# evanmayer/effex

Measured on AMD Instinct MI355X. Metric: 2-ant FX correlator throughput (PFB+FFT+X, integrated), higher is better.
Workload: dtype f32; 1 GPU; configs[1]: 2-antenna FX, num_samp=262144, ntaps=4, nchan=4096, 10000 integration frames per GPU per step; frames_per_gpu=10000, frames_total=10000, resident_frames=10000, num_samp=262144, nchan=4096, ntaps=4, n_ant=2, sample_definition=one complex sample per antenna stream, reduce_transport=none (single rank), library=effex_amd/csrc/libfxcorr.so

## Files before the change

### effex_amd/csrc/fx_fused4096.h

```cpp
#pragma once
#include "fx_math.h"

#if defined(__HIP_DEVICE_COMPILE__)
#define FXC_SCHED_FENCE() __builtin_amdgcn_sched_barrier(0)
#else
#define FXC_SCHED_FENCE() ((void)0)
#endif

namespace fxc {
namespace fused {

FX_HD cf lds_load(const cf* p) {
#if defined(__HIP_DEVICE_COMPILE__)
    typedef const volatile __attribute__((address_space(3))) unsigned long long* lds_u64_ptr;
    const unsigned long long u = *(lds_u64_ptr)(p);
    cf r;
    r.x = __uint_as_float((unsigned)(u & 0xffffffffull));
    r.y = __uint_as_float((unsigned)(u >> 32));
    return r;
#else
    return *p;
#endif
}

FX_HD f4 lds_load4(const f4* p) {
#if defined(__HIP_DEVICE_COMPILE__)
    typedef float lds_v4f __attribute__((ext_vector_type(4)));
    typedef const volatile __attribute__((address_space(3))) lds_v4f* lds_v4f_ptr;
    const lds_v4f u = *(lds_v4f_ptr)(p);
    f4 r;
    r.x = u[0]; r.y = u[1]; r.z = u[2]; r.w = u[3];
    return r;
#else
    return *p;
#endif
}

constexpr int kN = 4096;
constexpr int kT = 4;
constexpr int kThreads = 512;
constexpr int kPlaneRow = 288;
constexpr int kPlane = 16 * kPlaneRow;
constexpr int kAntPlanes = 2 * kPlane;
constexpr int kRegionBytes = 2 * kAntPlanes * 4;
constexpr int kAccPerThread = 8;
#ifndef FXC_FIR_GROUP
#define FXC_FIR_GROUP 4
#endif
constexpr int kFirGroup = FXC_FIR_GROUP;

constexpr int kLdsRegion = 0;
constexpr int kLdsWin = kLdsRegion + kRegionBytes;
constexpr int kLdsTw2 = kLdsWin + kN * 16;
constexpr int kLdsBytes = kLdsTw2 + 256 * 8;

FX_HD int branch_of_thread(int t) {
    const int l = t & 63, wv = (t >> 6) & 3;
    return ((l >> 1) & 15) + 16 * ((l & 1) | ((l >> 5) << 1) | (wv << 2));
}
FX_HD int thread_of_branch(int j) { return ((j >> 4) & 1) | ((j & 15) << 1) | (j & 0xE0); }

struct LaneStore {
#if defined(__HIP_DEVICE_COMPILE__)
    unsigned m0;
#else
    float* at;
#endif
};

FX_HD LaneStore lane_store_begin(cf* region, int base_dw, int lane) {
    LaneStore ls;
#if defined(__HIP_DEVICE_COMPILE__)
    typedef __attribute__((address_space(3))) cf* lptr_t;
    (void)lane;
    ls.m0 = __builtin_amdgcn_readfirstlane((unsigned)(size_t)(lptr_t)region + 4u * (unsigned)base_dw);
    asm volatile("s_nop 0" : : "{m0}"(ls.m0));
#else
    ls.at = reinterpret_cast<float*>(region) + base_dw + lane;
#endif
    return ls;
}

template <int DW>
FX_HD void lane_store(const LaneStore& ls, float val) {
    static_assert(DW >= 0 && 4 * DW < 65536, "16-bit immediate");
#if defined(__HIP_DEVICE_COMPILE__)
    asm volatile("ds_write_addtid_b32 %0 offset:%1" : : "v"(val), "n"(4 * DW), "{m0}"(ls.m0));
#else
    ls.at[DW] = val;
#endif
}

FX_HD void lane_store_end() {
#if defined(__HIP_DEVICE_COMPILE__)
    asm volatile("s_waitcnt lgkmcnt(0)" : : : "memory");
#endif
}

template <int K>
struct KConst { static constexpr int value = K; };
template <class Sink>
FX_HD void dft16_b_stream_ct(cf (&v)[16], Sink&& sink) {
    dft4(v[0], v[1], v[2], v[3]);
    sink(KConst<0>{}, v[0]); sink(KConst<4>{}, v[1]); sink(KConst<8>{}, v[2]); sink(KConst<12>{}, v[3]);
    dft4_scaled_c_bd(v[4], v[5], v[6], v[7]);
    sink(KConst<1>{}, v[4]); sink(KConst<5>{}, v[5]); sink(KConst<9>{}, v[6]); sink(KConst<13>{}, v[7]);
    dft4_bd_scaled(v[8], v[9], v[10], v[11]);
    sink(KConst<2>{}, v[8]); sink(KConst<6>{}, v[9]); sink(KConst<10>{}, v[10]); sink(KConst<14>{}, v[11]);
    dft4_scaled_c_bd(v[12], v[13], v[14], v[15]);
    sink(KConst<3>{}, v[12]); sink(KConst<7>{}, v[13]); sink(KConst<11>{}, v[14]); sink(KConst<15>{}, v[15]);
}

struct State {
    cf h[4][16];
    cf tw1[16];
    cf acc[kAccPerThread];
    cf tw2[16];
};

template <int PH>
FX_HD void state_reset_history(State& s) {
#pragma unroll
    for (int d = 1; d < 4; ++d)
#pragma unroll
        for (int r = 0; r < 16; ++r) s.h[(PH + d) & 3][r] = mk(0.f, 0.f);
}

FX_HD void state_reset_all(State& s) {
    state_reset_history<0>(s);
#pragma unroll
    for (int q = 0; q < kAccPerThread; ++q) s.acc[q] = mk(0.f, 0.f);
}

struct RangeWalk {
    int c, i;
    int left;
    int row;
    int n_pts;
    int seg, seg_left;
    int seg_jump;
    int unit, in_row;
    int row_step;
    int row_off;
    bool rows_are_chunks;
    bool lead;
};

struct RangeSplit {
    int rounds, n_full, n_tail, rows_rounds, n_rows;
};

FX_HD RangeSplit range_split(int g, int n_chunks, int seg, int unit, bool rows_are_chunks) {
    RangeSplit r;
    r.rounds = n_chunks / (g * seg);
    r.n_full = r.rounds * g * seg;
    r.n_tail = n_chunks - r.n_full;
    r.rows_rounds = rows_are_chunks ? r.n_full : g * ((r.rounds * seg + unit - 1) / unit);
    r.n_rows = r.rows_rounds + r.n_tail + g;
    return r;
}

FX_HD RangeWalk range_walk_rounds(int b, int g, int n_chunks, int n_pts, int seg,
                                   int unit, bool rows_are_chunks) {
    const RangeSplit sp = range_split(g, n_chunks, seg, unit, rows_are_chunks);
    RangeWalk w;
    w.c = b * seg;
    w.i = 0;
    w.left = sp.rounds * seg * n_pts;
    w.n_pts = n_pts;
    w.seg = w.seg_left = seg;
    w.seg_jump = (g - 1) * seg;
    w.unit = rows_are_chunks ? 1 : unit;
    w.in_row = 0;
    w.rows_are_chunks = rows_are_chunks;
    w.row_off = 0;
    w.row_step = g;
    w.row = rows_are_chunks ? w.c : b;
    w.lead = false;
    return w;
}

FX_HD RangeWalk range_walk_tail(int b, int g, int n_chunks, int n_pts, int seg,
                                 int unit, bool rows_are_chunks) {
    const RangeSplit sp = range_split(g, n_chunks, seg, unit, rows_are_chunks);
    RangeWalk w;
    const int n_frames = sp.n_tail * n_pts;
    const int f0 = range_begin(b, n_frames, g);
    w.left = range_begin(b + 1, n_frames, g) - f0;
    w.c = sp.n_full + f0 / n_pts;
    w.i = f0 % n_pts;
    w.n_pts = n_pts;
    w.seg = 1;
    w.seg_left = 1;
    w.seg_jump = 0;
    w.unit = 1;
    w.in_row = 0;
    w.rows_are_chunks = true;
    w.row_off = sp.rows_rounds - sp.n_full;
    w.row_step = 0;
    w.lead = w.i != 0;
    w.row = w.lead ? sp.rows_rounds + sp.n_tail + b : w.c + w.row_off;
    return w;
}

FX_HD bool range_walk_row_ends(const RangeWalk& w) {
    return w.left == 1 || (w.i + 1 == w.n_pts && w.in_row + 1 == w.unit);
}

FX_HD void range_walk_prefetch(const RangeWalk& w, int& pc, int& pi) {
    pc = w.c;
    pi = w.i;
    if (w.left > 1 && ++pi == w.n_pts) {
        pi = 0;
        pc += 1 + (w.seg_left == 1 ? w.seg_jump : 0);
    }
}

FX_HD void range_walk_advance(RangeWalk& w, bool row_ended) {
    if (++w.i == w.n_pts) {
        w.i = 0;
        w.c += 1;
        if (--w.seg_left == 0) {
            w.c += w.seg_jump;
            w.seg_left = w.seg;
        }
        w.in_row += 1;
    }
    w.left -= 1;
    if (row_ended) {
        w.in_row = 0;
        w.row = w.rows_are_chunks ? w.c + w.row_off : w.row + w.row_step;
    }
}

FX_HD int sample_offset(int j, int r) { return (kN - 1) - j - 256 * r; }

template <int PH, int G = kFirGroup, bool PIN = false>
FX_HD void phase1_fir_col(const State& s, const f4* win, int col, cf (&v)[16]) {
    const int j = col;
    const cf (&x0)[16] = s.h[PH];
    const cf (&x1)[16] = s.h[(PH + 3) & 3];
    const cf (&x2)[16] = s.h[(PH + 2) & 3];
    const cf (&x3)[16] = s.h[(PH + 1) & 3];
    constexpr int NG = 16 / G;
    f4 w[2][G];
#pragma unroll
    for (int q = 0; q < G; ++q) w[0][q] = PIN ? lds_load4(win + q * 256 + j) : win[q * 256 + j];
#pragma unroll
    for (int g = 0; g < NG; ++g) {
        if (g < NG - 1) {
#pragma unroll
            for (int q = 0; q < G; ++q) {
                const f4* at = win + (G * (g + 1) + q) * 256 + j;
                w[(g + 1) & 1][q] = PIN ? lds_load4(at) : *at;
            }
        }
        FXC_SCHED_FENCE();
#pragma unroll
        for (int q = 0; q < G; ++q) {
            const int r = G * g + q;
            const f4 t = w[g & 1][q];
            cf a = cscale(x0[r], t.x);
            a = cfma(t.y, x1[r], a);
            a = cfma(t.z, x2[r], a);
            v[r] = cfma(t.w, x3[r], a);
        }
#if defined(__HIP_DEVICE_COMPILE__)
        if (PIN) {
#pragma unroll
            for (int q = 0; q < G; ++q) asm volatile("" : "+v"(v[G * g + q].x), "+v"(v[G * g + q].y));
        }
#endif
        FXC_SCHED_FENCE();
    }
}

template <int PH, int G = kFirGroup>
FX_HD void phase1_fir(const State& s, const f4* win, int tid, cf (&v)[16]) {
    phase1_fir_col<PH, G>(s, win, tid & 255, v);
}

FX_HD cf tw1_of(const cf (&pw2)[4], int k1) {
    cf w = mk(1.f, 0.f);
    bool have = false;
#pragma unroll
    for (int b = 0; b < 4; ++b) {
        if (k1 & (1 << b)) {
            w = have ? cmul(w, pw2[b]) : pw2[b];
            have = true;
        }
    }
    return w;
}

template <bool LEAN_TW = false>
FX_HD void phase1_finish_store(const State& s, cf (&v)[16], cf* region, int tid) {
    const int t = thread_of_branch(tid & 255);
    const LaneStore ls = lane_store_begin(region, (tid >> 8) * kAntPlanes + (t & 0xC0), t & 63);
    cf pw2[4] = {s.tw1[1], s.tw1[2], s.tw1[4], s.tw1[8]};
#if defined(__HIP_DEVICE_COMPILE__)
    if (LEAN_TW) {
#pragma unroll
        for (int b = 0; b < 4; ++b) asm volatile("" : "+v"(pw2[b].x), "+v"(pw2[b].y));
    }
#endif
    dft16_b_stream_ct(v, [&](auto k, cf val) {
        constexpr int k1 = decltype(k)::value;
        if (k1 > 0) val = cmul(val, LEAN_TW ? tw1_of(pw2, k1) : s.tw1[k1]);
        lane_store<k1 * kPlaneRow>(ls, val.x);
        lane_store<kPlane + k1 * kPlaneRow>(ls, val.y);
    });
    lane_store_end();
}

FX_HD void state_load_twiddles(State& s, const cf* tw1_table, int tid) {
    const int j = tid & 255;
#pragma unroll
    for (int k1 = 0; k1 < 16; ++k1) s.tw1[k1] = tw1_table[k1 * 256 + j];
}

FX_HD void phase2_load(cf* region, int tid, cf (&v)[16]) {
    const int l = tid & 63, wave = tid >> 6;
    const int ant = l >> 5, k1 = 2 * wave + ((l >> 4) & 1), j0 = l & 15;
    const float* row = reinterpret_cast<const float*>(region) + ant * kAntPlanes + k1 * kPlaneRow + 2 * j0;
#pragma unroll
    for (int u = 0; u < 8; ++u) {
        const cf re = lds_load(reinterpret_cast<const cf*>(row + 32 * u));
        const cf im = lds_load(reinterpret_cast<const cf*>(row + kPlane + 32 * u));
        v[2 * u] = mk(re.x, im.x);
        v[2 * u + 1] = mk(re.y, im.y);
    }
}

FX_HD void phase2_twiddle(cf (&v)[16], const cf* tw2, int tid) {
    const int j0 = tid & 15;
    cf t[2][4];
#pragma unroll
    for (int q = 1; q < 4; ++q) t[0][q] = lds_load(tw2 + q * 16 + j0);
#pragma unroll
    for (int g = 0; g < 4; ++g) {
        if (g < 3) {
#pragma unroll
            for (int q = 0; q < 4; ++q) t[(g + 1) & 1][q] = lds_load(tw2 + (4 * (g + 1) + q) * 16 + j0);
        }
        FXC_SCHED_FENCE();
#pragma unroll
        for (int q = 0; q < 4; ++q) {
            const int q1 = 4 * g + q;
            if (q1 > 0) v[q1] = cmul(v[q1], t[g & 1][q]);
        }
        FXC_SCHED_FENCE();
    }
}

#ifndef FXC_TW2_RESIDENT
#define FXC_TW2_RESIDENT 10
#endif
constexpr int kTw2Resident = FXC_TW2_RESIDENT;
static_assert(kTw2Resident >= 0 && kTw2Resident <= 15, "q1 = 1 .. 15");
FX_HD void state_load_twiddles2(State& s, const cf* tw2_table, int tid) {
    const int j0 = tid & 15;
#pragma unroll
    for (int q1 = 1; q1 <= kTw2Resident; ++q1) s.tw2[q1] = tw2_table[q1 * 16 + j0];
}

FX_HD void phase2_twiddle_fetch(cf (&t)[16], const cf* tw2, int tid) {
    const int j0 = tid & 15;
#pragma unroll
    for (int q1 = kTw2Resident + 1; q1 < 16; ++q1) t[q1] = lds_load(tw2 + q1 * 16 + j0);
}

FX_HD cf cmul_tw(cf a, cf b) {
    return mk(__builtin_fmaf(a.x, b.x, -(a.y * b.y)), __builtin_fmaf(a.y, b.x, a.x * b.y));
}

FX_HD void phase2_twiddle_reg(cf (&v)[16], const State& s, const cf (&t)[16]) {
#pragma unroll
    for (int q1 = 1; q1 <= kTw2Resident; ++q1) v[q1] = cmul_tw(v[q1], s.tw2[q1]);
#pragma unroll
    for (int q1 = kTw2Resident + 1; q1 < 16; ++q1) v[q1] = cmul_tw(v[q1], t[q1]);
}

constexpr int kStripeHi = kPlane + 32;
constexpr int stripe_of(int q1) { return (q1 >> 3) * kStripeHi + (q1 & 7) * 66; }

template <int Q1>
FX_HD void phase2_store_from(const LaneStore& ls, const cf (&v)[16]) {
    lane_store<stripe_of(Q1)>(ls, v[Q1].x);
    lane_store<stripe_of(Q1) + kAntPlanes>(ls, v[Q1].y);
    if constexpr (Q1 < 15) phase2_store_from<Q1 + 1>(ls, v);
}

FX_HD void phase2_store(const cf (&v)[16], cf* region, int tid) {
    const LaneStore ls = lane_store_begin(region, (tid >> 6) * 2 * kPlaneRow, tid & 63);
    phase2_store_from<0>(ls, v);
    lane_store_end();
}

FX_HD void phase3_load(cf* region, int tid, cf (&v)[16]) {
    const int l = tid & 63, wave = tid >> 6, q1 = l & 15;
    const float* row = reinterpret_cast<const float*>(region) + wave * 2 * kPlaneRow + stripe_of(q1) + (l >> 4) * 16;
#pragma unroll
    for (int u = 0; u < 8; ++u) {
        const cf re = lds_load(reinterpret_cast<const cf*>(row + 2 * u));
        const cf im = lds_load(reinterpret_cast<const cf*>(row + kAntPlanes + 2 * u));
        v[2 * u] = mk(re.x, im.x);
        v[2 * u + 1] = mk(re.y, im.y);
    }
}

FX_HD void xacc(State& s, int q, cf a, cf b) { s.acc[q] = cmulc_acc(s.acc[q], a, b); }

FX_HD int bin_of(int tid, int q) {
    const int l = tid & 63, wave = tid >> 6;
    const int k1 = 2 * wave + ((l >> 4) & 1), q1 = l & 15, q2 = q + 8 * (l >> 5);
    return k1 + 16 * q1 + 256 * q2;
}

FX_HD int slot_of_bin(int k) {
    const int k1 = k & 15, q1 = (k >> 4) & 15, q2 = k >> 8;
    const int l = (q2 >> 3) * 32 + (k1 & 1) * 16 + q1;
    const int tid = (k1 >> 1) * 64 + l;
    return (q2 & 7) * kThreads + tid;
}

FX_HD int lane_specpos(int tid) {
    const int l = tid & 63, wave = tid >> 6;
    return (2 * wave + ((l >> 4) & 1)) * 16 + (l & 15);
}

FX_HD int specpos(int lane_l, int q2) { return (q2 >> 1) * 512 + 2 * lane_l + (q2 & 1); }
FX_HD int specpos_of_bin(int k) { return specpos((k & 15) * 16 + ((k >> 4) & 15), k >> 8); }

}
}
```

### effex_amd/csrc/k_fused4096.h

```cpp
#pragma once

namespace {

__device__ __forceinline__ void wave_sync() {
    __builtin_amdgcn_fence(__ATOMIC_RELEASE, "wavefront");
    __builtin_amdgcn_wave_barrier();
    __builtin_amdgcn_fence(__ATOMIC_ACQUIRE, "wavefront");
}

__device__ __forceinline__ void permlane32_swap(cf& a, cf& b) {
    auto rx = __builtin_amdgcn_permlane32_swap(__float_as_uint(a.x), __float_as_uint(b.x), false, false);
    auto ry = __builtin_amdgcn_permlane32_swap(__float_as_uint(a.y), __float_as_uint(b.y), false, false);
    a = fxc::mk(__uint_as_float(rx[0]), __uint_as_float(ry[0]));
    b = fxc::mk(__uint_as_float(rx[1]), __uint_as_float(ry[1]));
}

typedef unsigned v2u32 __attribute__((ext_vector_type(2)));
typedef unsigned v4u32 __attribute__((ext_vector_type(4)));
#ifndef FXC_LOAD_AUX_U8
#define FXC_LOAD_AUX_U8 2
#endif
#ifndef FXC_LOAD_AUX
#define FXC_LOAD_AUX 2
#endif
#ifndef FXC_PAIR_SOFF
#define FXC_PAIR_SOFF 1
#endif
struct FetchBase {
    const cf* base;
    __amdgpu_buffer_rsrc_t rs, rs_odd;
};
__device__ __forceinline__ void fetch_base_set(FetchBase& fb, const cf* chunk_base, unsigned chunk_bytes) {
    fb.base = chunk_base;
    fb.rs = __builtin_amdgcn_make_buffer_rsrc(const_cast<cf*>(chunk_base), 0, (int)chunk_bytes, 0x00020000);
    fb.rs_odd = __builtin_amdgcn_make_buffer_rsrc(const_cast<cf*>(chunk_base + 256), 0, (int)chunk_bytes, 0x00020000);
}

template <int R0, int CNT>
__device__ __forceinline__ void load_frame_part(cf (&xr)[16], const FetchBase& fb, unsigned voff, int64_t i) {
    const __amdgpu_buffer_rsrc_t rs = fb.rs, rs_odd = fb.rs_odd;
    const unsigned soff = (unsigned)(i * fxc::fused::kN * (int64_t)sizeof(cf));
    constexpr unsigned kRowBytes = 256 * sizeof(cf);
    static_assert(R0 % 2 == 0 && CNT % 2 == 0, "whole row pairs");
#pragma unroll
    for (int r = R0; r < R0 + CNT; ++r) {
        const int row = 15 - r, srow = FXC_PAIR_SOFF ? (row & ~1) : row;
        const v2u32 d = __builtin_amdgcn_raw_buffer_load_b64(row != srow ? rs_odd : rs, voff, soff + (unsigned)srow * kRowBytes, FXC_LOAD_AUX);
        xr[r] = fxc::mk(__uint_as_float(d[0]), __uint_as_float(d[1]));
    }
}
template <int R0, int CNT>
__device__ __forceinline__ void load_frame_part(cf (&xr)[16], const cf* chunk_base, unsigned chunk_bytes, unsigned voff,
                                                int64_t i) {
    FetchBase fb;
    fetch_base_set(fb, chunk_base, chunk_bytes);
    load_frame_part<R0, CNT>(xr, fb, voff, i);
}

template <int R0, int CNT>
__device__ __forceinline__ void load_frame_part_u8(cf (&xr)[16], const unsigned short* chunk_base,
                                                   unsigned chunk_bytes, unsigned voff, int64_t i) {
    __amdgpu_buffer_rsrc_t rs = __builtin_amdgcn_make_buffer_rsrc(const_cast<unsigned short*>(chunk_base), 0,
                                                                   (int)chunk_bytes, 0x00020000);
    const unsigned soff = (unsigned)(i * fxc::fused::kN * (int64_t)sizeof(unsigned short));
#pragma unroll
    for (int r = R0; r < R0 + CNT; ++r)
        xr[r].x = __uint_as_float(
            (unsigned)__builtin_amdgcn_raw_buffer_load_b16(rs, voff, soff + (unsigned)(256 * (15 - r) * sizeof(unsigned short)), FXC_LOAD_AUX_U8));
}

__device__ __forceinline__ void convert_frame_u8(cf (&h)[16], cf off) {
    const float k = 1.0f / 127.5f;
#pragma unroll
    for (int r = 0; r < 16; ++r) {
        const unsigned raw = __float_as_uint(h[r].x);
        h[r] = fxc::mk(fmaf((float)(raw & 0xFFu), k, off.x), fmaf((float)((raw >> 8) & 0xFFu), k, off.y));
    }
}

#ifndef FXC_ABL
#define FXC_ABL 0
#endif
#ifndef FXC_STAMPS
#define FXC_STAMPS 0
#endif
constexpr int kStampSegs = 12;
constexpr int kDckLdsBytes = 64;
constexpr int kAutoLdsBytes = fxc::fused::kAccPerThread * fxc::fused::kThreads * 4;
#if FXC_STAMPS
#define FXC_STAMP(k)                                                              \
    do {                                                                          \
        __builtin_amdgcn_sched_barrier(0);                                        \
        const unsigned long long t_now__ = __builtin_amdgcn_s_memtime();          \
        __builtin_amdgcn_s_waitcnt(0xC07F);                                       \
        seg[k] += t_now__ - t_prev;                                               \
        t_prev = t_now__;                                                         \
        __builtin_amdgcn_sched_barrier(0);                                        \
    } while (0)
#else
#define FXC_STAMP(k)
#endif
#if (FXC_ABL & 16)
#define FXC_PREFETCH(R0) ((void)0)
#else
#define FXC_PREFETCH(R0)                                                                                        \
    do {                                                                                                        \
        FXC_SCHED_FENCE();                                                                                      \
        if (U8)                                                                                                 \
            load_frame_part_u8<R0, 4>(nx, reinterpret_cast<const unsigned short*>(x) + (int64_t)pc * 2 * num_samp, \
                                      chunk_bytes, voff, nframe);                                               \
        else if (FXC_CARRY_BASE)                                                                                \
            load_frame_part<R0, 4>(nx, fb, voff, nframe);                                                       \
        else                                                                                                    \
            load_frame_part<R0, 4>(nx, x + (int64_t)pc * 2 * num_samp, chunk_bytes, voff, nframe);              \
        FXC_SCHED_FENCE();                                                                                      \
    } while (0)
#endif

struct U8State {
    cf off;
    bool have_next;
    bool rounds;
};

typedef unsigned v4u32_t __attribute__((ext_vector_type(4)));
constexpr int kDckStageVecs = 2 * fxc::fused::kThreads;

__device__ __forceinline__ void dck_fetch(const unsigned char* pair_base, int64_t num_samp, int64_t i, int tid, v4u32_t* stage) {
    typedef __attribute__((address_space(3))) v4u32_t* lptr_t;
    unsigned t = (unsigned)tid;
    asm volatile("" : "+v"(t));
    const unsigned lane_off = ((t >> 8) & 1u) * (unsigned)(2 * num_samp) + (t & 255u) * 16u;
    const unsigned char* base = pair_base + i * (fxc::fused::kThreads * 16);
    const unsigned lds_wave = __builtin_amdgcn_readfirstlane((unsigned)(size_t)(lptr_t)(stage + (t >> 6) * 128));
    unsigned m0_saved;
    asm volatile(
        "s_mov_b32 %[sv], m0\n\t"
        "s_mov_b32 m0, %[l0]\n\t"
        "s_nop 0\n\t"
        "global_load_lds_dwordx4 %[o0], %[base]\n\t"
        "s_add_u32 m0, %[l0], 0x400\n\t"
        "s_nop 0\n\t"
        "global_load_lds_dwordx4 %[o1], %[base]\n\t"
        "s_mov_b32 m0, %[sv]\n\t"
        : [sv] "=&s"(m0_saved)
        : [l0] "s"(lds_wave), [o0] "v"(lane_off), [o1] "v"(lane_off + 4096u), [base] "s"(base)
        : "memory", "scc");
}

__device__ __forceinline__ void dck_wait_prev() { asm volatile("s_waitcnt vmcnt(16)" ::: "memory"); }
__device__ __forceinline__ void dck_wait_own() { asm volatile("s_waitcnt vmcnt(4)" ::: "memory"); }

__device__ __forceinline__ void dck_clear(v4u32_t* stage, int tid) {
    unsigned z0;
    asm volatile("" : "+v"(tid));
    asm volatile("v_mov_b32 %0, 0" : "=v"(z0));
    const v4u32_t z = {z0, z0, z0, z0};
    stage[(tid >> 6) * 128 + (tid & 63)] = z;
    stage[(tid >> 6) * 128 + 64 + (tid & 63)] = z;
}

__device__ __forceinline__ void dck_add(const v4u32_t* stage, unsigned* acc, int tid) {
    asm volatile("" : "+v"(tid));
    unsigned si = 0u, sq = 0u;
#pragma unroll
    for (int h = 0; h < 2; ++h) {
        const v4u32_t w = stage[(tid >> 6) * 128 + h * 64 + (tid & 63)];
#pragma unroll
        for (int k = 0; k < 4; ++k) {
            si = __builtin_amdgcn_udot4(w[k], 0x00010001u, si, false);
            sq = __builtin_amdgcn_udot4(w[k], 0x01000100u, sq, false);
        }
    }
    acc[2 * tid] += si;
    acc[2 * tid + 1] += sq;
}

__device__ __forceinline__ cf dck_offset(unsigned* acc, unsigned* red, int tid, int64_t num_samp) {
    asm volatile("" : "+v"(tid));
    unsigned zero;
    asm volatile("v_mov_b32 %0, 0" : "=v"(zero));
    unsigned v[2] = {acc[2 * tid], acc[2 * tid + 1]};
    acc[2 * tid] = zero;
    acc[2 * tid + 1] = zero;
#pragma unroll
    for (int k = 0; k < 2; ++k) {
#pragma unroll
        for (int d = 32; d >= 1; d >>= 1) v[k] += __shfl_xor(v[k], d, 64);
    }
    __syncthreads();
    if ((tid & 63) == 0) {
        red[(tid >> 6) * 2] = v[0];
        red[(tid >> 6) * 2 + 1] = v[1];
    }
    __syncthreads();
    const int ant = (tid >> 8) & 1;
    unsigned long long ti = 0, tq = 0;
#pragma unroll
    for (int wv = 0; wv < 4; ++wv) {
        ti += red[(4 * ant + wv) * 2];
        tq += red[(4 * ant + wv) * 2 + 1];
    }
    asm volatile("" : "+s"(num_samp));
    const double mr = (double)ti / (double)num_samp, mi = (double)tq / (double)num_samp;
    return fxc::mk((float)(-mr / 127.5), (float)(-mi / 127.5));
}

#ifndef FXC_REG_TW2
#define FXC_REG_TW2 1
#endif
#ifndef FXC_CARRY_BASE
#define FXC_CARRY_BASE 1
#endif
#ifndef FXC_SPEC_STORE_AUX
#define FXC_SPEC_STORE_AUX 2
#endif
template <int PH, bool SPEC_OUT, bool U8, bool DCK, bool AUTOS>
__device__ __forceinline__ void fused_step(fxc::fused::State& s, float (&pw)[fxc::fused::kAccPerThread], float* pw_lds, U8State& u8, const cf* dc, const f4* win, cf* region,
                                           const cf* tw2, int tid, const cf* x, int64_t num_samp, unsigned chunk_bytes,
                                           unsigned voff, fxc::fused::RangeWalk& pos, FetchBase& fb, cf* rows_raw, int hp, v4u32_t* dck_stage,
                                           unsigned* dck_acc, unsigned* dck_red,
                                           unsigned long long (&seg)[kStampSegs], unsigned long long& t_prev) {
    using namespace fxc::fused;
    const int64_t c = pos.c, i = pos.i, n_pts = pos.n_pts;
    FXC_STAMP(0);
    if (i == 0) {
        asm volatile("" ::: "memory");
        state_reset_history<PH>(s);
        if (U8) {
            if (DCK && u8.have_next) u8.off = dck_offset(dck_acc, dck_red, tid, num_samp);
            else u8.off = dc[c * 2 + __builtin_amdgcn_readfirstlane((tid >> 8) & 1)];
        }
    }
    const bool dck_next = DCK && u8.rounds && pos.left > n_pts - i;
    const unsigned char* dck_base = reinterpret_cast<const unsigned char*>(x) + (int64_t)(c + (dck_next ? 1 + pos.seg_jump : 0)) * 4 * num_samp;
    if (U8) convert_frame_u8(s.h[PH], u8.off);
    cf v[16];
    constexpr bool REG_TW2 = FXC_REG_TW2 && !SPEC_OUT && !U8 && !DCK && !AUTOS;
    phase1_fir_col<PH, AUTOS ? 2 : kFirGroup, REG_TW2>(s, win, tid & 255, v);
    FXC_STAMP(2);
    int pc, nframe;
    range_walk_prefetch(pos, pc, nframe);
    if (FXC_CARRY_BASE && !U8 && pc != pos.c) {
        asm volatile("" ::: "memory");
        fetch_base_set(fb, fb.base + (int64_t)(pc - pos.c) * 2 * num_samp, chunk_bytes);
    }
    cf (&nx)[16] = s.h[(PH + 1) & 3];
    FXC_PREFETCH(0);
    fxc::dft16_a(v);
    FXC_PREFETCH(4);
    FXC_STAMP(3);
#if !(FXC_ABL & 1)
    __syncthreads();
#endif
    FXC_STAMP(4);
#if !(FXC_ABL & 4)
    phase1_finish_store<AUTOS>(s, v, region, (tid & ~255) | branch_of_thread(tid & 255));
#endif
    FXC_STAMP(5);
#if !(FXC_ABL & 2)
    __syncthreads();
#endif
    if (DCK) {
        dck_wait_prev();
        dck_add(dck_stage, dck_acc, tid);
        dck_fetch(dck_base, num_samp, i, tid, dck_stage);
    }
    FXC_STAMP(6);
    cf tw2_late[16];
    if (REG_TW2) phase2_twiddle_fetch(tw2_late, tw2, tid);
#if !(FXC_ABL & 4)
    phase2_load(region, tid, v);
#endif
    FXC_PREFETCH(8);
    fxc::dft16(v);
    FXC_STAMP(7);
    if (REG_TW2) phase2_twiddle_reg(v, s, tw2_late);
    else phase2_twiddle(v, tw2, tid);
    FXC_STAMP(8);
#if !(FXC_ABL & 8)
    wave_sync();
    phase2_store(v, region, tid);
    wave_sync();
#endif
    FXC_PREFETCH(12);
#if !(FXC_ABL & 8)
    phase3_load(region, tid, v);
#endif
    FXC_STAMP(9);
    fxc::dft16(v);
    if (SPEC_OUT) {
        const unsigned cu = (unsigned)c;
        const unsigned cr = hp == 1 ? cu : (hp == 2 ? cu >> 1 : (hp == 4 ? cu >> 2 : (unsigned)(((unsigned long long)cu * 0xAAAAAAABull) >> 33)));
        const int64_t row0 = ((int64_t)cr * n_pts + i) * (2 * hp) + 2 * (cu - cr * hp);
        __amdgpu_buffer_rsrc_t rs = __builtin_amdgcn_make_buffer_rsrc(rows_raw + row0 * kN, 0, (int)(2 * kN * (int64_t)sizeof(cf)), 0x00020000);
        const unsigned voff0 = (unsigned)(((tid >> 5) & 1) * kN + specpos(lane_specpos(tid), 0)) * (unsigned)sizeof(cf);
#pragma unroll
        for (int m = 0; m < 8; ++m) {
            v4u32 d = {__float_as_uint(v[2 * m].x), __float_as_uint(v[2 * m].y), __float_as_uint(v[2 * m + 1].x),
                       __float_as_uint(v[2 * m + 1].y)};
            __builtin_amdgcn_raw_buffer_store_b128(d, rs, voff0 + (unsigned)(m * 512 * sizeof(cf)), 0, FXC_SPEC_STORE_AUX);
        }
    } else {
#pragma unroll
        for (int q = 0; q < 8; ++q) {
            cf a = v[q], b = v[q + 8];
            permlane32_swap(a, b);
            xacc(s, q, a, b);
            if (AUTOS) {
                pw[q] = __builtin_fmaf(a.y, a.y, __builtin_fmaf(a.x, a.x, pw[q]));
                float* p1 = pw_lds + q * kThreads + tid;
                *p1 = __builtin_fmaf(b.y, b.y, __builtin_fmaf(b.x, b.x, *p1));
            }
        }
        FXC_STAMP(10);
    }
    if (DCK) {
        if (i + 1 == n_pts) {
            dck_wait_own();
            dck_add(dck_stage, dck_acc, tid);
            dck_clear(dck_stage, tid);
        }
        u8.have_next = dck_next;
    }
    const bool row_ends = !SPEC_OUT && range_walk_row_ends(pos);
    if (row_ends) {
        if (DCK) {
            __amdgpu_buffer_rsrc_t rs = __builtin_amdgcn_make_buffer_rsrc(rows_raw + (int64_t)pos.row * kN, 0, (int)(kN * (int64_t)sizeof(cf)), 0x00020000);
            unsigned t = (unsigned)tid;
            asm volatile("" : "+v"(t));
#pragma unroll
            for (int q = 0; q < kAccPerThread; ++q) {
                const v2u32 d = {__float_as_uint(s.acc[q].x), __float_as_uint(s.acc[q].y)};
                __builtin_amdgcn_raw_buffer_store_b64(d, rs, t * (unsigned)sizeof(cf), (unsigned)(q * kThreads * sizeof(cf)), 0);
                s.acc[q] = fxc::mk(0.f, 0.f);
            }
        } else {
            cf* row = rows_raw + (int64_t)pos.row * (AUTOS ? 3 : 1) * kN + tid;
#pragma unroll
            for (int q = 0; q < kAccPerThread; ++q) {
                row[q * kThreads] = s.acc[q];
                s.acc[q] = fxc::mk(0.f, 0.f);
                if (AUTOS) {
                    row[kN + q * kThreads] = fxc::mk(pw[q], 0.f);
                    row[2 * kN + q * kThreads] = fxc::mk(pw_lds[q * kThreads + tid], 0.f);
                    pw[q] = pw_lds[q * kThreads + tid] = 0.f;
                }
            }
        }
    }
    range_walk_advance(pos, row_ends);
}

template <bool SPEC_OUT, bool U8 = false, bool DCK = false, bool AUTOS = false>
__global__ __launch_bounds__(fxc::fused::kThreads, 2) void fx_fused4096_kernel(
    const cf* __restrict__ x, int64_t num_samp, int64_t n_pts, int64_t n_chunks, const f4* __restrict__ win_g,
    const cf* __restrict__ tw1_g, const cf* __restrict__ tw2_g, cf* __restrict__ rows_raw,
    unsigned long long* __restrict__ stamps, const cf* __restrict__ dc, int seg, int unit, int rows_are_chunks) {
    using namespace fxc::fused;
    extern __shared__ __attribute__((aligned(16))) unsigned char smem[];
    f4* win = reinterpret_cast<f4*>(smem + kLdsWin);
    cf* region = reinterpret_cast<cf*>(smem + kLdsRegion);
    cf* tw2 = reinterpret_cast<cf*>(smem + kLdsTw2);

    const int tid = threadIdx.x;
    const int ant = tid >> 8, j = branch_of_thread(tid & 255);
    for (int idx = tid; idx < kN; idx += kThreads) win[idx] = win_g[(idx & ~255) | branch_of_thread(idx & 255)];
    if (tid < 256) tw2[tid] = tw2_g[tid];
    State s;
    state_load_twiddles(s, tw1_g, (ant << 8) | j);
    if (FXC_REG_TW2 && !SPEC_OUT && !U8 && !DCK && !AUTOS) state_load_twiddles2(s, tw2_g, tid);
#pragma unroll
    for (int q = 0; q < kAccPerThread; ++q) s.acc[q] = fxc::mk(0.f, 0.f);
    static_assert(!AUTOS || (!SPEC_OUT && !U8), "autos: the complex64 F+X variant only");
    float pw[kAccPerThread];
    float* pw_lds = reinterpret_cast<float*>(smem + kLdsBytes);
#pragma unroll
    for (int q = 0; q < kAccPerThread; ++q) {
        pw[q] = 0.f;
        if (AUTOS) pw_lds[q * kThreads + tid] = 0.f;
    }
    __syncthreads();

    constexpr int64_t kSampleBytes = U8 ? sizeof(unsigned short) : sizeof(cf);
    const unsigned voff = (unsigned)((ant * num_samp + (255 - j)) * kSampleBytes);
    const unsigned chunk_bytes = (unsigned)(2 * num_samp * kSampleBytes);
    static_assert(!DCK || (U8 && !SPEC_OUT), "in-kernel DC removal: uint8 ingest only");
    U8State u8;
    u8.off = fxc::mk(0.f, 0.f);
    u8.have_next = u8.rounds = false;
    __shared__ v4u32_t dck_stage_mem[DCK ? kDckStageVecs : 1];
    __shared__ unsigned dck_acc_mem[DCK ? 2 * kThreads : 1];
    v4u32_t* dck_stage = dck_stage_mem;
    unsigned* dck_acc = dck_acc_mem;
    unsigned* dck_red = reinterpret_cast<unsigned*>(smem + kLdsBytes);
    if (DCK) {
        dck_acc[2 * tid] = dck_acc[2 * tid + 1] = 0u;
        dck_clear(dck_stage, tid);
    }
    unsigned long long seg_t[kStampSegs] = {0, 0, 0, 0, 0, 0, 0, 0, 0, 0, 0, 0};
    unsigned long long t_prev = 0;
    int64_t frames_done = 0;
#if FXC_STAMPS
    t_prev = __builtin_amdgcn_s_memtime();
#endif
#pragma unroll 1
    for (int part = 0; part < 2; ++part) {
        const int walk_unit = SPEC_OUT ? 1 : unit;
        int np_walk = (int)n_pts, seg_walk = seg, unit_walk = walk_unit;
        if (DCK) asm volatile("" : "+s"(np_walk), "+s"(seg_walk), "+s"(unit_walk));
        RangeWalk pos = part == 0 ? range_walk_rounds(blockIdx.x, gridDim.x, (int)n_chunks, np_walk, seg_walk, unit_walk, rows_are_chunks != 0)
                                  : range_walk_tail(blockIdx.x, gridDim.x, (int)n_chunks, np_walk, seg_walk, unit_walk, rows_are_chunks != 0);
        const int total = pos.left;
        if (!SPEC_OUT && part == 1 && (!pos.lead || total == 0)) {
            const RangeSplit sp = range_split(gridDim.x, (int)n_chunks, seg, walk_unit, rows_are_chunks != 0);
            int t_lead = tid;
            if (DCK) asm volatile("" : "+v"(t_lead));
            cf* lead_row = rows_raw + (int64_t)(sp.rows_rounds + sp.n_tail + blockIdx.x) * (AUTOS ? 3 : 1) * kN + t_lead;
#pragma unroll
            for (int q = 0; q < (AUTOS ? 3 : 1) * kAccPerThread; ++q) lead_row[q * kThreads] = fxc::mk(0.f, 0.f);
        }
        if (total == 0) continue;
        if (U8) u8.off = dc[(int64_t)pos.c * 2 + __builtin_amdgcn_readfirstlane(ant)];
        u8.have_next = false;
        u8.rounds = part == 0;
        const cf* cbase = reinterpret_cast<const cf*>(reinterpret_cast<const char*>(x) + (int64_t)pos.c * 2 * num_samp * kSampleBytes);
#pragma unroll
        for (int d = 1; d < 4; ++d) {
            if (pos.i - d >= 0) {
                if (U8) {
                    load_frame_part_u8<0, 16>(s.h[4 - d], reinterpret_cast<const unsigned short*>(cbase), chunk_bytes, voff, pos.i - d);
                    convert_frame_u8(s.h[4 - d], u8.off);
                } else {
                    load_frame_part<0, 16>(s.h[4 - d], cbase, chunk_bytes, voff, pos.i - d);
                }
            } else {
#pragma unroll
                for (int r = 0; r < 16; ++r) s.h[4 - d][r] = fxc::mk(0.f, 0.f);
            }
        }
        if (U8)
            load_frame_part_u8<0, 16>(s.h[0], reinterpret_cast<const unsigned short*>(cbase), chunk_bytes, voff, pos.i);
        else
            load_frame_part<0, 16>(s.h[0], cbase, chunk_bytes, voff, pos.i);
        FetchBase fb;
        fetch_base_set(fb, cbase, chunk_bytes);
#pragma unroll 1
        for (int g = 0; g < total; g += 4) {
            fused_step<0, SPEC_OUT, U8, DCK, AUTOS>(s, pw, pw_lds, u8, dc, win, region, tw2, tid, x, num_samp, chunk_bytes, voff, pos, fb, rows_raw, SPEC_OUT ? unit : 0, dck_stage, dck_acc, dck_red, seg_t, t_prev);
            if (g + 1 < total)
                fused_step<1, SPEC_OUT, U8, DCK, AUTOS>(s, pw, pw_lds, u8, dc, win, region, tw2, tid, x, num_samp, chunk_bytes, voff, pos, fb, rows_raw, SPEC_OUT ? unit : 0, dck_stage, dck_acc, dck_red, seg_t, t_prev);
            if (g + 2 < total)
                fused_step<2, SPEC_OUT, U8, DCK, AUTOS>(s, pw, pw_lds, u8, dc, win, region, tw2, tid, x, num_samp, chunk_bytes, voff, pos, fb, rows_raw, SPEC_OUT ? unit : 0, dck_stage, dck_acc, dck_red, seg_t, t_prev);
            if (g + 3 < total)
                fused_step<3, SPEC_OUT, U8, DCK, AUTOS>(s, pw, pw_lds, u8, dc, win, region, tw2, tid, x, num_samp, chunk_bytes, voff, pos, fb, rows_raw, SPEC_OUT ? unit : 0, dck_stage, dck_acc, dck_red, seg_t, t_prev);
        }
        frames_done += total;
    }
#if FXC_STAMPS
    if (stamps && (tid & 63) == 0) {
        unsigned long long* dst = stamps + ((int64_t)blockIdx.x * (kThreads / 64) + (tid >> 6)) * kStampSegs;
        for (int k = 0; k < kStampSegs; ++k) dst[k] = seg_t[k];
        dst[kStampSegs - 1] = (unsigned long long)frames_done;
    }
#else
    (void)stamps;
    (void)frames_done;
#endif
}

}
```

Baseline: 311,400 Msamples/s.

## Add explicit group waitcnts and interleave twiddle multiply with LDS stores

Replaces compiler-inserted full waits in the FIR phase with staged s_waitcnt values, so each group of four FIR rows waits only for its own loads. The twiddle multiply is interleaved with the per-lane LDS stores to overlap ALU work with DS writes. The initial frame load is split into four scheduled parts followed by an explicit entry wait, so the counters line up with the staged waits. Hand-encoded waitcnt values depend on the exact instruction order and could be wrong if the compiler reorders loads.

```diff
diff --git a/effex_amd/csrc/fx_fused4096.h b/effex_amd/csrc/fx_fused4096.h
--- a/effex_amd/csrc/fx_fused4096.h
+++ b/effex_amd/csrc/fx_fused4096.h
@@ -94,6 +94,14 @@
 FX_HD void lane_store_end() {
 #if defined(__HIP_DEVICE_COMPILE__)
     asm volatile("s_waitcnt lgkmcnt(0)" : : : "memory");
+#endif
+}
+
+template <int VM, int LGKM>
+FX_HD void group_wait() {
+    static_assert(VM >= 0 && VM < 64 && LGKM >= 0 && LGKM < 16, "6 bits of vmcnt, 4 of lgkmcnt");
+#if defined(__HIP_DEVICE_COMPILE__)
+    __builtin_amdgcn_s_waitcnt((VM & 15) | ((VM >> 4) << 14) | (7 << 4) | (LGKM << 8));
 #endif
 }
 
@@ -235,8 +243,9 @@
 
 FX_HD int sample_offset(int j, int r) { return (kN - 1) - j - 256 * r; }
 
-template <int PH, int G = kFirGroup, bool PIN = false>
+template <int PH, int G = kFirGroup, bool PIN = false, bool GW = false>
 FX_HD void phase1_fir_col(const State& s, const f4* win, int col, cf (&v)[16]) {
+    static_assert(!GW || (PIN && G == 4), "group waits: written for pinned groups of four");
     const int j = col;
     const cf (&x0)[16] = s.h[PH];
     const cf (&x1)[16] = s.h[(PH + 3) & 3];
@@ -256,6 +265,13 @@
             }
         }
         FXC_SCHED_FENCE();
+        if (GW) {
+            if (g == 0) group_wait<12, 4>();
+            else if (g == 1) group_wait<8, 4>();
+            else if (g == 2) group_wait<4, 4>();
+            else group_wait<0, 0>();
+            FXC_SCHED_FENCE();
+        }
 #pragma unroll
         for (int q = 0; q < G; ++q) {
             const int r = G * g + q;
@@ -391,6 +407,22 @@
     if constexpr (Q1 < 15) phase2_store_from<Q1 + 1>(ls, v);
 }
 
+template <int Q1>
+FX_HD void phase2_twiddle_store_from(const LaneStore& ls, cf (&v)[16], const State& s, const cf (&t)[16]) {
+    if constexpr (Q1 > 0) v[Q1] = cmul_tw(v[Q1], Q1 <= kTw2Resident ? s.tw2[Q1] : t[Q1]);
+    lane_store<stripe_of(Q1)>(ls, v[Q1].x);
+    lane_store<stripe_of(Q1) + kAntPlanes>(ls, v[Q1].y);
+    FXC_SCHED_FENCE();
+    if constexpr (Q1 < 15) phase2_twiddle_store_from<Q1 + 1>(ls, v, s, t);
+}
+
+FX_HD void phase2_twiddle_store(cf (&v)[16], const State& s, const cf (&t)[16], cf* region, int tid) {
+    const LaneStore ls = lane_store_begin(region, (tid >> 6) * 2 * kPlaneRow, tid & 63);
+    FXC_SCHED_FENCE();
+    phase2_twiddle_store_from<0>(ls, v, s, t);
+    lane_store_end();
+}
+
 FX_HD void phase2_store(const cf (&v)[16], cf* region, int tid) {
     const LaneStore ls = lane_store_begin(region, (tid >> 6) * 2 * kPlaneRow, tid & 63);
     phase2_store_from<0>(ls, v);
diff --git a/effex_amd/csrc/k_fused4096.h b/effex_amd/csrc/k_fused4096.h
--- a/effex_amd/csrc/k_fused4096.h
+++ b/effex_amd/csrc/k_fused4096.h
@@ -212,6 +212,15 @@
 #ifndef FXC_CARRY_BASE
 #define FXC_CARRY_BASE 1
 #endif
+#ifndef FXC_X2_STORE_AMONG_TW
+#define FXC_X2_STORE_AMONG_TW 1
+#endif
+#ifndef FXC_GROUP_WAITS
+#define FXC_GROUP_WAITS 1
+#endif
+#ifndef FXC_ENTRY_WAIT
+#define FXC_ENTRY_WAIT 1
+#endif
 #ifndef FXC_SPEC_STORE_AUX
 #define FXC_SPEC_STORE_AUX 2
 #endif
@@ -236,8 +245,11 @@
     const unsigned char* dck_base = reinterpret_cast<const unsigned char*>(x) + (int64_t)(c + (dck_next ? 1 + pos.seg_jump : 0)) * 4 * num_samp;
     if (U8) convert_frame_u8(s.h[PH], u8.off);
     cf v[16];
-    constexpr bool REG_TW2 = FXC_REG_TW2 && !SPEC_OUT && !U8 && !DCK && !AUTOS;
-    phase1_fir_col<PH, AUTOS ? 2 : kFirGroup, REG_TW2>(s, win, tid & 255, v);
+    constexpr bool DEFAULT_INST = !SPEC_OUT && !U8 && !DCK && !AUTOS;
+    constexpr bool REG_TW2 = FXC_REG_TW2 && DEFAULT_INST;
+    constexpr bool X2_AMONG_TW = FXC_X2_STORE_AMONG_TW && REG_TW2 && !(FXC_ABL & 8);
+    constexpr bool GROUP_WAITS = FXC_GROUP_WAITS && REG_TW2 && kFirGroup == 4;
+    phase1_fir_col<PH, AUTOS ? 2 : kFirGroup, REG_TW2, GROUP_WAITS>(s, win, tid & 255, v);
     FXC_STAMP(2);
     int pc, nframe;
     range_walk_prefetch(pos, pc, nframe);
@@ -275,14 +287,21 @@
     FXC_PREFETCH(8);
     fxc::dft16(v);
     FXC_STAMP(7);
-    if (REG_TW2) phase2_twiddle_reg(v, s, tw2_late);
-    else phase2_twiddle(v, tw2, tid);
-    FXC_STAMP(8);
+    if (X2_AMONG_TW) {
+        FXC_STAMP(8);
+        wave_sync();
+        phase2_twiddle_store(v, s, tw2_late, region, tid);
+        wave_sync();
+    } else {
+        if (REG_TW2) phase2_twiddle_reg(v, s, tw2_late);
+        else phase2_twiddle(v, tw2, tid);
+        FXC_STAMP(8);
 #if !(FXC_ABL & 8)
-    wave_sync();
-    phase2_store(v, region, tid);
-    wave_sync();
-#endif
+        wave_sync();
+        phase2_store(v, region, tid);
+        wave_sync();
+#endif
+    }
     FXC_PREFETCH(12);
 #if !(FXC_ABL & 8)
     phase3_load(region, tid, v);
@@ -420,7 +439,7 @@
 #pragma unroll
             for (int q = 0; q < (AUTOS ? 3 : 1) * kAccPerThread; ++q) lead_row[q * kThreads] = fxc::mk(0.f, 0.f);
         }
-        if (total == 0) continue;
+        if (total <= 0) continue;
         if (U8) u8.off = dc[(int64_t)pos.c * 2 + __builtin_amdgcn_readfirstlane(ant)];
         u8.have_next = false;
         u8.rounds = part == 0;
@@ -439,12 +458,29 @@
                 for (int r = 0; r < 16; ++r) s.h[4 - d][r] = fxc::mk(0.f, 0.f);
             }
         }
-        if (U8)
-            load_frame_part_u8<0, 16>(s.h[0], reinterpret_cast<const unsigned short*>(cbase), chunk_bytes, voff, pos.i);
-        else
-            load_frame_part<0, 16>(s.h[0], cbase, chunk_bytes, voff, pos.i);
         FetchBase fb;
         fetch_base_set(fb, cbase, chunk_bytes);
+        constexpr bool DEFAULT_INST = !SPEC_OUT && !U8 && !DCK && !AUTOS;
+        if (U8) {
+            load_frame_part_u8<0, 16>(s.h[0], reinterpret_cast<const unsigned short*>(cbase), chunk_bytes, voff, pos.i);
+        } else if ((FXC_GROUP_WAITS || FXC_ENTRY_WAIT) && DEFAULT_INST) {
+            FXC_SCHED_FENCE();
+            load_frame_part<0, 4>(s.h[0], fb, voff, pos.i);
+            FXC_SCHED_FENCE();
+            load_frame_part<4, 4>(s.h[0], fb, voff, pos.i);
+            FXC_SCHED_FENCE();
+            load_frame_part<8, 4>(s.h[0], fb, voff, pos.i);
+            FXC_SCHED_FENCE();
+            load_frame_part<12, 4>(s.h[0], fb, voff, pos.i);
+            FXC_SCHED_FENCE();
+        } else {
+            load_frame_part<0, 16>(s.h[0], cbase, chunk_bytes, voff, pos.i);
+        }
+        if (FXC_ENTRY_WAIT && DEFAULT_INST) {
+            FXC_SCHED_FENCE();
+            group_wait<16, 15>();
+            FXC_SCHED_FENCE();
+        }
 #pragma unroll 1
         for (int g = 0; g < total; g += 4) {
             fused_step<0, SPEC_OUT, U8, DCK, AUTOS>(s, pw, pw_lds, u8, dc, win, region, tw2, tid, x, num_samp, chunk_bytes, voff, pos, fb, rows_raw, SPEC_OUT ? unit : 0, dck_stage, dck_acc, dck_red, seg_t, t_prev);
```

Result: no change. 313,700 Msamples/s (median of 3 runs) (+0.7%).
